# RaulPPelaez/UAMMD

Measured on AMD Instinct MI355X. Metric: particle-steps/s (LJ 1e6, rho*=0.8) + FCM-BDHI steps/s @128^3, 1/2/4/8 GPU, higher is better.
Workload: dtype f32

## Files before the change

### uammd_amd/csrc/fcm.hip

```cpp
#include "ibm.hpp"
#include "celllist.hpp"
#include "rocfft_plans.hpp"
#include "saru.hpp"

#include <cmath>
#include <string>

namespace uammd_hip {

struct PseGreens { float rh, split, eta, shear; bool on; };

struct FcmPrep {
  int4 *origin;
  float *weights;
  float4 *force;
  int *tileOf;
  int *rank;
  int *tileCount;
  int *tileStart;
  int wstride;
  int3 tdim;
  unsigned long long *rec;
  int *ovfTile;
  int cap;
  int *slotCount;
  int *slotCountNext;
  int *slotFlag;
  const float4 *forceById;
};

struct FCM {
  uammd_fcm_parameters par;
  GridT<float> grid;
  IBMKernelDev kern;
  IBMKernelDev kernT{};
  bool haveTorqueKernel = false;
  int nxpad = 0;
  size_t planeReal = 0;
  size_t planeCplx = 0;
  DeviceBuffer gridBuf, gridBufT, interBuf, prepOrigin, prepWeights, prepTileOf, prepRank, prepTileCount, prepTileStart, prepSorted;
  int emVelN = 0;
  DeviceBuffer emVel;
  bool emBin = true;
  bool binnedPending = false;
  const void *binnedPos = nullptr;
  int binnedN = 0;
  bool useTiles = false;
  int3 ntiles{0, 0, 0};
  int3 tdim{8, 8, 8};
  int prepCapN = 0;
  bool tileCountZero = false;
  DeviceBuffer prepRec, prepOvfTile, prepSlotCount;
  bool slotsEnabled = !(getenv("UAMMD_FCM_SLOTS") && atoi(getenv("UAMMD_FCM_SLOTS")) == 0);
  int slotCap = 0;
  int slotParity = 0;
  bool slotPending = false;
  bool slotDirty = true;
  const void *slotPos = nullptr;
  int slotN = 0;
  int slotRefresh = 128;
  bool lastSolveSlots = false;
  int orderN = 0;
  int slotSteps = 0;
  int *slotFlagHost = nullptr, *slotFlagDev = nullptr;
  bool binBySlot = true;
  hipStream_t prepStream = nullptr;
  bool prepStreamSet = false;
  bool forceAtomicSpread = false;
  bool interGather = true;
  int gatherPerWave = 2;
  int spreadWaves = 0;
  bool tileGather = false;
  bool accumulate = false;
  int zTileLog2 = 0;
  bool customFFT = true;
  PseGreens pse{0.f, 0.f, 0.f, 0.f, false};
  RealFFT fft;
  unsigned int seed2 = 0;
  FcmPrep halfPrep{};
  int halfN = 0;
  bool halfPending = false;
  ~FCM() {
    if (slotFlagHost) (void)hipHostFree(slotFlagHost);
  }
};
// ... 176 lines not shown
  const int3 P = compute_support_shift(grid, pi, celli, kern.support);
  const int ox = celli.x - P.x, oy = celli.y - P.y, oz = celli.z - P.z;
  const int slot = pr.tileStart[pr.tileOf[id]] + pr.rank[id];
  float *w = pr.weights + (size_t)pr.wstride * slot;
  const int sx = kern.support.x, sy = kern.support.y, sz = kern.support.z;
  for (int k = sub; k < sx + sy + sz; k += LANES) {
    float v;
    if (k < sx) v = phi_axis(kern, 0, grid.distanceToCellCenter(pi, make_int3(grid.pbc_x(ox + k), celli.y, celli.z)).x);
    else if (k < sx + sy) v = phi_axis(kern, 1, grid.distanceToCellCenter(pi, make_int3(celli.x, grid.pbc_y(oy + k - sx), celli.z)).y);
    else v = phi_axis(kern, 2, grid.distanceToCellCenter(pi, make_int3(celli.x, celli.y, grid.pbc_z(oz + k - sx - sy))).z);
    w[k] = v;
  }
  if (sub) return;
  pr.origin[slot] = make_int4(ox, oy, oz, id);
  float4 fr = force ? force[id] : make_float4(0.f, 0.f, 0.f, 0.f);
  int rel;
  (void)stencil_tile(ox, oy, oz, grid.cellDim, pr.tdim, make_int3(1, 1, 1), &rel);
  fr.w = __int_as_float(rel);
  pr.force[slot] = fr;
}

template <int KIND, int LANES>
__global__ void __launch_bounds__(256) k_fcm_step_prep(float4 *__restrict__ pos, const float *__restrict__ linearV, int N, float dt,
                                                        GridT<float> grid, IBMKernelDev kern, int3 ntiles, FcmPrep pr, int ovfCap) {
  kern.kind = KIND;
  const int gid = blockIdx.x * 256 + threadIdx.x;
  const int s = gid / LANES, sub = gid % LANES;
  const bool live = s < N;
  const bool head = live && sub == 0;
  const int id = live ? pr.origin[s].w : 0;
  float4 p = pos[id];
  if (linearV) {
    p.x = fmaf(linearV[3 * id], dt, p.x);
    p.y = fmaf(linearV[3 * id + 1], dt, p.y);
    p.z = fmaf(linearV[3 * id + 2], dt, p.z);
    if (head) pos[id] = p;
  }
  const real3f pi{p.x, p.y, p.z};
  const int3 celli = grid.getCell(pi);
  const int3 P = compute_support_shift(grid, pi, celli, kern.support);
  const int ox = celli.x - P.x, oy = celli.y - P.y, oz = celli.z - P.z;
  int rel;
  const int t = stencil_tile(ox, oy, oz, grid.cellDim, pr.tdim, ntiles, &rel);
  const int lane = threadIdx.x & 63;
  unsigned long long rem = __ballot(head);
  int cnt = 1, before = 0, lead = lane;
  for (int round = 0; round < 8 && rem; ++round) {
    const int l = __ffsll((unsigned long long)rem) - 1;
    const int t0 = __builtin_amdgcn_readlane(t, l);
    const unsigned long long m = __ballot(head && t == t0) & rem;
    if (head && t == t0 && ((rem >> lane) & 1ull)) {
      cnt = __popcll(m);
      before = __popcll(m & ((1ull << lane) - 1ull));
      lead = l;
    }
    rem &= ~m;
  }
  int got = 0;
  if (head && lane == lead) got = atomicAdd(&pr.slotCount[t], cnt);
  if ((blockIdx.x & 15) == 0 && threadIdx.x < 64) {
// ... 562 lines not shown
        if (wsel[r] >= 0) {
          ax[q] = fmaf(dV, v[q][r].x * wx * wy * wz, ax[q]);
          ay[q] = fmaf(dV, v[q][r].y * wx * wy * wz, ay[q]);
          az[q] = fmaf(dV, v[q][r].z * wx * wy * wz, az[q]);
        }
      }
    }
  }
#pragma unroll
  for (int o2 = 32; o2 > 0; o2 >>= 1) {
#pragma unroll
    for (int q = 0; q < P; ++q) {
      ax[q] += __shfl_xor(ax[q], o2, 64);
      ay[q] += __shfl_xor(ay[q], o2, 64);
      az[q] += __shfl_xor(az[q], o2, 64);
    }
  }
  if (lane == 0) {
#pragma unroll
    for (int q = 0; q < P; ++q) {
      if (slot0 + q >= N) break;
      float *out = vout + 3 * (size_t)o[q].w;
      if (accumulate) { out[0] += ax[q]; out[1] += ay[q]; out[2] += az[q]; } else { out[0] = ax[q]; out[1] = ay[q]; out[2] = az[q]; }
    }
  }
}
template <int P, int SZMAX>
__global__ void __launch_bounds__(64 * kGatherWaves) k_fcm_gather_col(float *__restrict__ vout, const float4 *__restrict__ gi, int N, int3 n,
                                                                      int3 support, float dV, FcmPrep pr, bool accumulate) {
  const int lane = threadIdx.x & 63;
  const int slot0 = ((int)xcd_contiguous_block(blockIdx.x, gridDim.x) * kGatherWaves + (threadIdx.x >> 6)) * P;
  if (slot0 >= N) return;
  const int sx = support.x, sy = support.y, sz = support.z;
  const int ii = lane & 7, jj = lane >> 3;
  const bool col = ii < sx && jj < sy;
  int4 o[P];
  float wl[P];
#pragma unroll
  for (int q = 0; q < P; ++q) {
    const int slot = min(slot0 + q, N - 1);
    o[q] = pr.origin[slot];
    wl[q] = pr.weights[(size_t)pr.wstride * slot + min(lane, sx + sy + sz - 1)];
  }
  float4 g[P][SZMAX];
  float wxy[P];
  const uint planeNodes = (uint)n.x * (uint)n.y;
// ... 24 lines not shown
        const float wz = __builtin_bit_cast(float, __builtin_amdgcn_readlane(__builtin_bit_cast(int, wl[q]), sx + sy + kk));
        const float w = wxy[q] * wz;
        if (col) {
          ax[q] = fmaf(g[q][kk].x, w, ax[q]);
          ay[q] = fmaf(g[q][kk].y, w, ay[q]);
          az[q] = fmaf(g[q][kk].z, w, az[q]);
        }
      }
    }
  }
#pragma unroll
  for (int q = 0; q < P; ++q) {
    ax[q] = wave_total(ax[q]);
    ay[q] = wave_total(ay[q]);
    az[q] = wave_total(az[q]);
  }
  if (lane == 0) {
#pragma unroll
    for (int q = 0; q < P; ++q) {
      if (slot0 + q >= N) break;
      ax[q] *= dV; ay[q] *= dV; az[q] *= dV;
      float *out = vout + 3 * (size_t)o[q].w;
      if (accumulate) { out[0] += ax[q]; out[1] += ay[q]; out[2] += az[q]; } else { out[0] = ax[q]; out[1] = ay[q]; out[2] = az[q]; }
    }
  }
}
template <int S, int SZMAX>
__global__ void __launch_bounds__(64 * kGatherWaves) k_fcm_gather_half(float *__restrict__ vout, const float4 *__restrict__ gi, int N, int3 n,
                                                                       int sz, float dV, FcmPrep pr, bool accumulate) {
  constexpr int R = S * S - 32;
  constexpr int ROUNDS = (R * SZMAX + 31) / 32;
  static_assert(R > 0 && 2 * S + SZMAX <= 32, "supports 6 and 7");
  const int lane = threadIdx.x & 63, h = lane >> 5, l = lane & 31;
  const int slot0 = ((int)xcd_contiguous_block(blockIdx.x, gridDim.x) * kGatherWaves + (threadIdx.x >> 6)) * 2;
  if (slot0 >= N) return;
  const bool valid = slot0 + h < N;
  const int slot = min(slot0 + h, N - 1);
  const int4 o = pr.origin[slot];
  const float wl = pr.weights[(size_t)pr.wstride * slot + min(l, 2 * S + sz - 1)];
  const int jj = l / S, ii = l - S * jj;
  const uint planeNodes = (uint)n.x * (uint)n.y;
  auto wrap = [](int c, int m) { return c < 0 ? c + m : (c >= m ? c - m : c); };
  const uint base = (uint)wrap(o.x + ii, n.x) + (uint)n.x * (uint)wrap(o.y + jj, n.y);
  float4 g[SZMAX];
#pragma unroll
  for (int kk = 0; kk < SZMAX; ++kk)
// ... 33 lines not shown
    const bool rest = kk2[r] >= 0;
    const float w = __shfl(wl, hb + ii2[r], 64) * __shfl(wl, hb + S + jj2[r], 64) * __shfl(wl, hb + 2 * S + (rest ? kk2[r] : 0), 64);
    if (rest) {
      ax = fmaf(g2[r].x, w, ax);
      ay = fmaf(g2[r].y, w, ay);
      az = fmaf(g2[r].z, w, az);
    }
  }
  auto half_sum = [](float x) {
    x += dpp_move<0xB1, 0xf, true>(x);
    x += dpp_move<0x4E, 0xf, true>(x);
    x += dpp_move<0x141, 0xf, true>(x);
    x += dpp_move<0x140, 0xf, true>(x);
    x += dpp_move<0x142, 0xa, false>(x);
    return x;
  };
  ax = half_sum(ax);
  ay = half_sum(ay);
  az = half_sum(az);
  if (l == 31 && valid) {
    ax *= dV; ay *= dV; az *= dV;
    float *out = vout + 3 * (size_t)o.w;
    if (accumulate) { out[0] += ax; out[1] += ay; out[2] += az; } else { out[0] = ax; out[1] = ay; out[2] = az; }
  }
}
static void launch_gather_inter(hipStream_t st, float *vout, const float4 *gi, int N, int3 n, int3 support, float dV, FastDiv dsx,
                                FastDiv dsxy, const FcmPrep &pr, bool accumulate, int perWave = 2, bool packed = false) {
  const size_t nodes = (size_t)n.x * n.y * n.z;
  static const int halfMode = getenv("UAMMD_FCM_GATHER_HALF") ? atoi(getenv("UAMMD_FCM_GATHER_HALF")) : 1;
  if (packed) {
    const int rounds = (support.x * support.y * support.z + 63) / 64;
    const int P = rounds <= 4 ? (perWave >= 4 ? 4 : 2) : 1;
    const dim3 g((N + kGatherWaves * P - 1) / (kGatherWaves * P)), b(64 * kGatherWaves);
#define UH_GIP(RR, PP) hipLaunchKernelGGL((k_fcm_gather_inter<RR, PP, true>), g, b, 0, st, vout, gi, N, n, support, dV, dsx, dsxy, pr, accumulate)
    if (rounds <= 1) UH_GIP(1, 2); else if (rounds <= 2) UH_GIP(2, 2); else if (rounds <= 4) { if (P == 4) UH_GIP(4, 4); else UH_GIP(4, 2); } else UH_GIP(8, 1);
#undef UH_GIP
    return;
  }
  if (halfMode == 2 && perWave >= 0 && support.x == 6 && support.y == 6 && support.z <= 8 && nodes * sizeof(float4) < ((size_t)1 << 32)) {
    const dim3 g((N + kGatherWaves * 2 - 1) / (kGatherWaves * 2)), b(64 * kGatherWaves);
    if (support.z <= 6) hipLaunchKernelGGL((k_fcm_gather_half<6, 6>), g, b, 0, st, vout, gi, N, n, support.z, dV, pr, accumulate);
    else hipLaunchKernelGGL((k_fcm_gather_half<6, 8>), g, b, 0, st, vout, gi, N, n, support.z, dV, pr, accumulate);
    return;
  }
  if (perWave >= 0 && support.x <= 8 && support.y <= 8 && support.z <= 8 && nodes * sizeof(float4) <= ((size_t)128 << 20)) {
    constexpr int P = 2;
// ... 203 lines not shown
  if (t >= total) return;
  const uint tq = lay.divNkx.div((uint)t);
  const uint tz = lay.divNyl.div(tq);
  const int3 cell = make_int3(t - (int)tq * nkx, lay.y0 + (int)(tq - tz * (uint)lay.nyl), (int)tz);
  const int id = cell.x + nkx * (cell.y + nk.y * cell.z);
  const size_t a0 = (size_t)cell.x + (size_t)nkx * (size_t)(cell.y - lay.y0) + lay.zStride * (size_t)cell.z;
  float2 *g1 = g0 + lay.compStride, *g2 = g0 + 2 * lay.compStride;
  C3 in{0.f, 0.f, 0.f, 0.f, 0.f, 0.f};
  if (haveForce && id != 0) {
    const float2 a = g0[a0], b = g1[a0], c = g2[a0];
    in = C3{a.x, a.y, b.x, b.y, c.x, c.y};
  }
  const C3 v = fcm_kspace_node(cell, id, nk, nkx, L, viscosity, haveForce, noisePrefactor, seed1, seed2, pse, in);
  g0[a0] = make_float2(v.xr, v.xi);
  g1[a0] = make_float2(v.yr, v.yi);
  g2[a0] = make_float2(v.zr, v.zi);
}

#include "fcm_fft.hpp"

template <int LOG2TL, int NT, bool P2>
__global__ void __launch_bounds__(NT) k_fft_z_fused(float2 *__restrict__ g, size_t planeC, size_t zStride, int nyl, int y0, int nzArg,
                                                    int3 nk, real3f L, float viscosity, bool haveForce, float noisePrefactor,
                                                    uint seed1, uint seed2, PseGreens pse) {
  extern __shared__ float2 lds[];
  constexpr int TL = 1 << LOG2TL, JG = NT >> LOG2TL, MAXB = 6 * 256 / NT;
  const int nz = fft_len<P2>(nzArg);
  const int LS = nz + 1, nkx = nk.x / 2 + 1;
  float2 *tw = lds, *buf = lds + nz;
  const int tid = threadIdx.x, l = tid & (TL - 1), jg = tid >> LOG2TL;
  const size_t slab = zStride;
  const int q0 = (int)xcd_contiguous_block(blockIdx.x, gridDim.x) * TL, nl = min(TL, nyl * nkx - q0);
  float2 *base = g + q0 + l;
  fft_twiddles<NT>(tw, nz, tid);
  constexpr int NLINES = 3 * TL, QF = 3 * 512 / NT, QL = 2 * 512 / NT;
  const int log2N = 31 - __builtin_clz((unsigned)nz);
  const bool edges = P2 && haveForce && nl == TL && log2N % 3 != 0 && log2N >= 5 && NLINES * (nz >> 2) <= QF * NT &&
                     NLINES * (nz >> 3) <= QL * NT;
  if (edges) {
    const int per = nz >> 2, total = NLINES * per;
    float2 v[QF][4];
#pragma unroll
    for (int q = 0; q < QF; ++q) {
      const int b = tid + q * NT;
      if (b < total) {
        const int j = b / NLINES, line = b - j * NLINES, c = line >> LOG2TL, ll = line & (TL - 1);
        const float2 *src = g + q0 + ll + (size_t)c * planeC + (size_t)j * slab;
#pragma unroll
        for (int r = 0; r < 4; ++r) v[q][r] = src[(size_t)(r * per) * slab];
      }
    }
#pragma unroll
    for (int q = 0; q < QF; ++q) {
      const int b = tid + q * NT;
      if (b < total) {
        const int j = b / NLINES, line = b - j * NLINES;
        fft_butterfly<4, -1>(v[q]);
        float2 *dst = buf + line * LS + 4 * j;
#pragma unroll
        for (int r = 0; r < 4; ++r) dst[r] = v[q][r];
      }
    }
    __syncthreads();
    fft_lds_p2_inner<-1, MAXB, NT>(buf, LS, log2N, NLINES, tw, 1, tid, true, false);
  } else if (haveForce) {
    if (l < nl) {
      const int perC = (nz + JG - 1) / JG;
      staged_copy<12, float2>(0, 3 * perC, 1,
          [&](int e) {
            const int c = e / perC, j = jg + (e - c * perC) * JG;
            return j < nz ? base[(size_t)c * planeC + (size_t)j * slab] : make_float2(0.f, 0.f);
          },
          [&](int e, float2 v) {
            const int c = e / perC, j = jg + (e - c * perC) * JG;
            if (j < nz) buf[(c * nl + l) * LS + j] = v;
          });
    }
    __syncthreads();
    fft_lds<-1, MAXB, NT, P2>(buf, LS, nz, 3 * nl, tw, 1, tid);
  } else
    __syncthreads();
  if (l < nl) {
    const int q = q0 + l, yl = q / nkx, kx = q - yl * nkx, ky = y0 + yl;
    for (int j = jg; j < nz; j += JG) {
      const int3 cell = make_int3(kx, ky, j);
      const int id = kx + nkx * (ky + nk.y * j);
      C3 in{0.f, 0.f, 0.f, 0.f, 0.f, 0.f};
      float2 *px = buf + l * LS + j, *py = buf + (nl + l) * LS + j, *pz = buf + (2 * nl + l) * LS + j;
      if (haveForce) in = C3{px->x, px->y, py->x, py->y, pz->x, pz->y};
      const C3 v = fcm_kspace_node(cell, id, nk, nkx, L, viscosity, haveForce, noisePrefactor, seed1, seed2, pse, in);
      *px = make_float2(v.xr, v.xi);
      *py = make_float2(v.yr, v.yi);
      *pz = make_float2(v.zr, v.zi);
    }
  }
  __syncthreads();
  if (edges) {
    fft_lds_p2_inner<1, MAXB, NT>(buf, LS, log2N, NLINES, tw, 1, tid, false, true);
    const int per = nz >> 3, total = NLINES * per;
#pragma unroll
    for (int q = 0; q < QL; ++q) {
      const int b = tid + q * NT;
      if (b < total) {
        const int j = b / NLINES, line = b - j * NLINES, c = line >> LOG2TL, ll = line & (TL - 1);
        const float2 *p = buf + line * LS + j;
        float2 v[8];
#pragma unroll
        for (int r = 0; r < 8; ++r) v[r] = p[r * per];
#pragma unroll
        for (int r = 1; r < 8; ++r) v[r] = ctw<1>(v[r], tw[j * r]);
        fft_butterfly<8, 1>(v);
        float2 *dst = g + q0 + ll + (size_t)c * planeC + (size_t)j * slab;
#pragma unroll
        for (int r = 0; r < 8; ++r) dst[(size_t)(r * per) * slab] = v[r];
      }
    }
    return;
  }
  fft_lds<1, MAXB, NT, P2>(buf, LS, nz, 3 * nl, tw, 1, tid);
  if (l < nl)
    for (int c = 0; c < 3; ++c)
      for (int j = jg; j < nz; j += JG) base[(size_t)c * planeC + (size_t)j * slab] = buf[(c * nl + l) * LS + j];
}

template <bool ACC>
__global__ void __launch_bounds__(256) k_fcm_half_curl(const float2 *__restrict__ in, float2 *__restrict__ out, size_t planeC,
                                                        int3 nk, real3f L, FastDiv divNkx, FastDiv divNy) {
  const int id = blockIdx.x * 256 + threadIdx.x;
  const int nkx = nk.x / 2 + 1;
  if (id >= nk.z * nk.y * nkx) return;
  const uint tq = divNkx.div((uint)id), tz = divNy.div(tq);
  const int cx = id - (int)tq * nkx, cy = (int)(tq - tz * (uint)nk.y), cz = (int)tz;
  const int3 ik = make_int3(cx - nk.x * (cx >= nkx), cy - nk.y * (cy >= nk.y / 2 + 1), cz - nk.z * (cz >= nk.z / 2 + 1));
  const real3f dk = gradient_fourier(ik, nk, wavevector(ik, L));
  const float2 gx = in[id], gy = in[planeC + id], gz = in[2 * planeC + id];
  const float h = 0.5f;
  float2 cxv = make_float2(h * fmaf(-dk.y, gz.y, dk.z * gy.y), h * fmaf(dk.y, gz.x, -(dk.z * gy.x)));
  float2 cyv = make_float2(h * fmaf(-dk.z, gx.y, dk.x * gz.y), h * fmaf(dk.z, gx.x, -(dk.x * gz.x)));
  float2 czv = make_float2(h * fmaf(-dk.x, gy.y, dk.y * gx.y), h * fmaf(dk.x, gy.x, -(dk.y * gx.x)));
  if (ACC) {
    const float2 ox = out[id], oy = out[planeC + id], oz = out[2 * planeC + id];
    cxv.x += ox.x; cxv.y += ox.y; cyv.x += oy.x; cyv.y += oy.y; czv.x += oz.x; czv.y += oz.y;
  }
  out[id] = cxv;
  out[planeC + id] = cyv;
// ... 67 lines not shown
  else
    hipLaunchKernelGGL((k_fft_x_r2c<false, false>), dim3((nrows + rows - 1) / rows), dim3(kFftThreads), sizeof(float2) * (size_t)(nx + rows * (nh + 1)), st, g,
                       nx, nrows, rows, (const float *)nullptr, (const float *)nullptr, 0);
  const int tiles = (nkx + 15) / 16;
  fft_launch_lines<-1>((float2 *)g, ny, nkx, 3 * nz, st);
  (void)tiles;
  return 0;
}
#ifndef UAMMD_ZG_THREADS
#define UAMMD_ZG_THREADS 256
#endif
static int fcm_fft_z_fused_launch(FCM *f, float2 *g, size_t planeC, size_t zStride, int nyl, int y0, int3 cells, real3f L, bool haveForce,
                                  float noisePrefactor, uint seed2, hipStream_t st) {
  const int nz = cells.z, nkx = cells.x / 2 + 1, lines = nyl * nkx;
  int ltl = nz <= 256 ? 3 : 2;
  if (f->zTileLog2 > 0 && sizeof(float2) * (size_t)(nz + 3 * (1 << f->zTileLog2) * (nz + 1)) <= 64 * 1024) ltl = f->zTileLog2;
  const int tlz = 1 << ltl;
  const size_t ldsz = sizeof(float2) * (size_t)(nz + 3 * tlz * (nz + 1));
  const dim3 gz((lines + tlz - 1) / tlz), bz(512);
#ifndef UAMMD_ZP_THREADS
#define UAMMD_ZP_THREADS 512
#endif
#define UH_ZFUSED(LT, P) hipLaunchKernelGGL((k_fft_z_fused<LT, UAMMD_ZP_THREADS, P>), gz, dim3(UAMMD_ZP_THREADS), ldsz, st, g, planeC, zStride, nyl, y0, nz, cells, L, f->par.viscosity, \
                                         haveForce, noisePrefactor, f->par.seed, seed2, f->pse)
  if (is_pow2(nz)) { if (ltl == 4) UH_ZFUSED(4, true); else if (ltl == 3) UH_ZFUSED(3, true); else UH_ZFUSED(2, true); }
  else {
#define UH_ZFUSED_G(LT) hipLaunchKernelGGL((k_fft_z_fused<LT, UAMMD_ZG_THREADS, false>), gz, dim3(UAMMD_ZG_THREADS), ldsz, st, g, planeC, zStride, nyl, y0, nz, \
                                           cells, L, f->par.viscosity, haveForce, noisePrefactor, f->par.seed, seed2, f->pse)
    if (ltl == 4) UH_ZFUSED_G(4); else if (ltl == 3) UH_ZFUSED_G(3); else UH_ZFUSED_G(2);
#undef UH_ZFUSED_G
  }
#undef UH_ZFUSED
  return 0;
}
static int fcm_fft_z_operator_y(FCM *f, float *g, bool haveForce, float noisePrefactor, hipStream_t st) {
  const int nx = f->grid.cellDim.x, ny = f->grid.cellDim.y, nz = f->grid.cellDim.z, nkx = nx / 2 + 1;
  const real3f L{f->par.boxSize[0], f->par.boxSize[1], f->par.boxSize[2]};
  if (int e = fcm_fft_z_fused_launch(f, (float2 *)g, f->planeCplx, (size_t)ny * nkx, ny, 0, f->grid.cellDim, L, haveForce, noisePrefactor, f->seed2, st)) return e;
  fft_launch_lines<1>((float2 *)g, ny, nkx, 3 * nz, st);
  return 0;
}
static bool fcm_inter_packed(const FCM *f) {
  static const bool on = !(getenv("UAMMD_FCM_PACKED_INTER") && atoi(getenv("UAMMD_FCM_PACKED_INTER")) == 0);
  const size_t nodes = (size_t)f->grid.cellDim.x * f->grid.cellDim.y * f->grid.cellDim.z;
  return on && nodes * sizeof(float4) > ((size_t)128 << 20) && f->gatherPerWave >= 0;
}
static int fcm_fft_inverse_x(FCM *f, float *g, float4 *inter, hipStream_t st, bool packed = false) {
  const int nx = f->grid.cellDim.x, ny = f->grid.cellDim.y, nz = f->grid.cellDim.z, nh = nx / 2;
  const int rows = std::max(1, std::min(8, 2048 / (3 * nh))), nrows = ny * nz;
  if (is_pow2(nx) && is_pow2(ny))
    hipLaunchKernelGGL(k_fft_x_c2r<true>, dim3((nrows + rows - 1) / rows), dim3(kFftThreads), sizeof(float2) * (size_t)(nx + 3 * rows * (nh + 1)), st,
                       g, f->planeReal, (size_t)ny * f->nxpad, ny, nx, nrows, rows, inter, packed ? -1 : 0, (size_t)0);
  else
    hipLaunchKernelGGL(k_fft_x_c2r<false>, dim3((nrows + rows - 1) / rows), dim3(kFftThreads), sizeof(float2) * (size_t)(nx + 3 * rows * (nh + 1)), st,
                       g, f->planeReal, (size_t)ny * f->nxpad, ny, nx, nrows, rows, inter, packed ? -1 : 0, (size_t)0);
  return 0;
}

static int fcm_prepare_tiles(FCM *f, const float *d_pos, const float *d_force, int N, hipStream_t st, FcmPrep *out, bool positionsKept = false) {
  const int nt = f->ntiles.x * f->ntiles.y * f->ntiles.z;
  const int wstride = f->kern.support.x + f->kern.support.y + f->kern.support.z;
  if (f->slotPending) {
    f->slotPending = false;
    f->slotDirty = true;
  }
  f->slotSteps = 0;
  if (f->prepCapN < N) {
    UH_CHECK(hipStreamSynchronize(st));
    f->orderN = 0;
    if (int e = f->prepOrigin.reserve(sizeof(int4) * (size_t)N)) return e;
    if (int e = f->prepWeights.reserve(sizeof(float) * (size_t)wstride * N)) return e;
    if (int e = f->prepSorted.reserve(sizeof(float4) * (size_t)N)) return e;
    if (int e = f->prepTileOf.reserve(sizeof(int) * (size_t)N)) return e;
    if (int e = f->prepRank.reserve(sizeof(int) * (size_t)N)) return e;
    if (int e = f->prepTileCount.reserve(sizeof(int) * (size_t)nt)) return e;
    f->tileCountZero = false;
    if (int e = f->prepTileStart.reserve(sizeof(int) * ((size_t)nt + 1))) return e;
    f->prepCapN = N;
  }
  FcmPrep pr{(int4 *)f->prepOrigin.ptr, (float *)f->prepWeights.ptr, (float4 *)f->prepSorted.ptr,
             (int *)f->prepTileOf.ptr, (int *)f->prepRank.ptr, (int *)f->prepTileCount.ptr,
             (int *)f->prepTileStart.ptr, wstride, f->tdim};
  if (f->prepStreamSet && f->prepStream != st) {
    UH_CHECK(hipStreamSynchronize(f->prepStream));
    f->tileCountZero = false;
  }
  const bool binned = f->binnedPending && positionsKept && f->binnedPos == (const void *)d_pos && f->binnedN == N && f->prepStream == st;
  if (f->binnedPending && !binned) f->tileCountZero = false;
  f->binnedPending = false;
// ... 192 lines not shown
  if (!h) { set_last_error("uammd_fcm_displacements: null argument"); return -1; }
  if (N <= 0) return 0;
  if (!d_pos || (!d_linearVelocity && stage == 0)) { set_last_error("uammd_fcm_displacements: null argument"); return -1; }
  FCM *f = reinterpret_cast<FCM *>(h);
  hipStream_t st = (hipStream_t)stream;
  float *g = (float *)f->gridBuf.ptr;
  const dim3 gp((N + 3) / 4), bp(256);
  const FastDiv dsx = make_fastdiv(f->kern.support.x), dsxy = make_fastdiv(f->kern.support.x * f->kern.support.y);
  if (int e = f->fft.set_stream((void *)st)) return e;
  const size_t zs = (size_t)f->nxpad * f->grid.cellDim.y;
  const bool tiles = f->useTiles && !f->forceAtomicSpread;
  const bool custom = stage == 0 && fcm_custom_fft_usable(f);
  FcmPrep pr{};
  bool slots = false;
  if (half != 2) f->halfPending = false;
  if (half == 2) {
    if (!f->halfPending || f->halfN != N) { set_last_error("uammd_fcm: the second half of a solve without its first"); return -1; }
    pr = f->halfPrep;
    f->halfPending = false;
  } else if (tiles) {
    if (int e = fcm_prepare_best(f, d_pos, d_force, N, st, positionsKept, &pr, &slots)) return e;
  }
  if (half != 2) f->lastSolveSlots = slots;
  if (d_force && half != 2) {
    if (tiles) {
      const int nt = f->ntiles.x * f->ntiles.y * f->ntiles.z;
      const int ww = spread_weight_words(N, f->ntiles, f->kern.support, f->tdim);
      const int sw = spread_waves(N, f->ntiles, f->kern.support, f->tdim, f->spreadWaves);
      const int edge = spread_edge(f->tdim);
      const dim3 sg(nt), sb(64 * sw);
      const size_t lds = spread_lds_bytes(ww, sw, edge);
#define UH_SPREAD(W, S, E) hipLaunchKernelGGL((k_fcm_spread_tile<W, S, E>), sg, sb, lds, st, g, f->grid.cellDim, f->nxpad, f->planeReal, zs, f->kern.support, f->ntiles, pr, ww)
      static const bool specOn = getenv("UAMMD_FCM_NO_SPEC") == nullptr;
      const bool eight = (f->kern.support.x - 2 + f->tdim.x) / f->tdim.x == 1 && (f->kern.support.y - 2 + f->tdim.y) / f->tdim.y == 1 &&
                         (f->kern.support.z - 2 + f->tdim.z) / f->tdim.z == 1;
      static const bool specDense = getenv("UAMMD_FCM_SPEC_DENSE") != nullptr;
      const bool spec = specOn && slots && eight && pr.cap >= 8 * sw && ww / (3 * edge) >= 64 * sw && (sw == 2 || specDense);
#define UH_SPREAD_SPEC(W, E) hipLaunchKernelGGL((k_fcm_spread_tile<W, true, E, true>), sg, sb, lds, st, g, f->grid.cellDim, f->nxpad, f->planeReal, zs, f->kern.support, f->ntiles, pr, ww)
      if (spec) {
        if (sw == 2) { if (edge == kTileMax) UH_SPREAD_SPEC(2, kTileMax); else UH_SPREAD_SPEC(2, kTile); }
        else { if (edge == kTileMax) UH_SPREAD_SPEC(4, kTileMax); else UH_SPREAD_SPEC(4, kTile); }
      }
      else if (edge == kTileMax) {
        if (sw == 2) { if (slots) UH_SPREAD(2, true, kTileMax); else UH_SPREAD(2, false, kTileMax); }
        else { if (slots) UH_SPREAD(4, true, kTileMax); else UH_SPREAD(4, false, kTileMax); }
      } else {
// ... 36 lines not shown
                       f->grid.cellDim, real3f{f->par.boxSize[0], f->par.boxSize[1], f->par.boxSize[2]}, f->par.viscosity,
                       d_force != nullptr, noisePrefactor, f->par.seed, f->seed2, f->pse);
    if (stage == 1) { UH_CHECK(hipGetLastError()); return 0; }
    if (int e = f->fft.inverse(g)) return e;
  }
  const bool interPath = tiles && f->interGather && !(tiles && (f->kern.support.x <= 6 && f->kern.support.y <= 6 && f->kern.support.z <= 6) && f->tileGather);
  if (custom && !interPath) { if (int e = fcm_fft_inverse_x(f, g, nullptr, st)) return e; }
  const bool smallSupport = f->kern.support.x <= 6 && f->kern.support.y <= 6 && f->kern.support.z <= 6;
  if (tiles && smallSupport && f->tileGather)
    hipLaunchKernelGGL(k_fcm_gather_tile, dim3(f->ntiles.x * f->ntiles.y * f->ntiles.z), bp, 0, st, d_linearVelocity,
                       (const float *)g, f->grid.cellDim, f->nxpad, f->planeReal, zs, f->kern.support, f->ntiles,
                       f->grid.cellVolume, dsx, dsxy, pr, f->accumulate);
  else if (tiles && f->interGather) {
    const size_t nodes = (size_t)f->grid.cellDim.x * f->grid.cellDim.y * f->grid.cellDim.z;
    if (int e = f->interBuf.reserve(sizeof(float4) * nodes)) return e;
    const bool packed = custom && fcm_inter_packed(f);
    if (custom) {
      if (int e = fcm_fft_inverse_x(f, g, (float4 *)f->interBuf.ptr, st, packed)) return e;
    } else
      hipLaunchKernelGGL(k_fcm_interleave, dim3((unsigned)((nodes + 255) / 256)), bp, 0, st, (const float *)g, f->grid.cellDim, f->nxpad,
                         f->planeReal, zs, (float4 *)f->interBuf.ptr);
    launch_gather_inter(st, d_linearVelocity, (const float4 *)f->interBuf.ptr, N, f->grid.cellDim, f->kern.support, f->grid.cellVolume,
                        dsx, dsxy, pr, f->accumulate, f->gatherPerWave, packed);
  } else if (tiles)
    hipLaunchKernelGGL(k_fcm_gather_prep, gp, bp, 0, st, d_linearVelocity, (const float *)g, N, f->grid.cellDim, f->nxpad,
                       f->planeReal, zs, f->kern.support, f->grid.cellVolume, dsx, dsxy, pr, f->accumulate);
  else
    hipLaunchKernelGGL((k_fcm_ibm<false>), gp, bp, 0, st, (const float4 *)d_pos, (const float4 *)nullptr,
                       d_linearVelocity, g, N, f->grid, f->nxpad, f->planeReal, zs, f->kern, dsx, dsxy, f->accumulate);
  UH_CHECK(hipGetLastError());
  return 0;
}

int uammd_fcm_displacements_staged(uammd_fcm *h, const float *d_pos, const float *d_force, int N, float temperature,
                                   float prefactor, float *d_linearVelocity, int stage, void *stream) {
  return fcm_displacements_impl(h, d_pos, d_force, N, temperature, prefactor, d_linearVelocity, stage, stream, false);
}

static bool fcm_step_prep_launch(FCM *f, float *d_pos, const float *v, int N, float dt, hipStream_t st, int *rc) {
  *rc = 0;
  if (f->slotFlagHost && f->slotFlagHost[0]) {
    f->slotsEnabled = false;
    return false;
  }
  if (f->slotSteps >= f->slotRefresh) { f->slotSteps = 0; return false; }
  if (v && fcm_entries_scrambled(f, N)) return false;
// ... 14 lines not shown
    if (int e = f->prepRec.reserve(recBytes)) return fail(e);
    if (int e = f->prepOvfTile.reserve(sizeof(int) * (size_t)N)) return fail(e);
    if (int e = f->prepSlotCount.reserve(sizeof(int) * 2 * ((size_t)nt + 2))) return fail(e);
    f->slotCap = cap;
    f->slotDirty = true;
  }
  int *counts = (int *)f->prepSlotCount.ptr;
  int parity;
  if (f->lastSolveSlots && !f->slotDirty) parity = f->slotParity ^ 1;
  else {
    if (hipMemsetAsync(counts, 0, sizeof(int) * 2 * ((size_t)nt + 2), st) != hipSuccess) return fail(-1);
    f->slotDirty = false;
    parity = 0;
  }
  FcmPrep pr{};
  pr.origin = (int4 *)f->prepOrigin.ptr;
  pr.weights = (float *)f->prepWeights.ptr;
  pr.wstride = f->kern.support.x + f->kern.support.y + f->kern.support.z;
  pr.tdim = f->tdim;
  pr.rec = (unsigned long long *)f->prepRec.ptr;
  pr.ovfTile = (int *)f->prepOvfTile.ptr;
  pr.cap = cap;
  pr.slotCount = counts + (size_t)parity * (nt + 2);
#define UH_STEP_PREP(K)                                                                                                                        \
  case K:                                                                                                                                      \
    if (N <= kPrepLanesUpTo)                                                                                                                   \
      hipLaunchKernelGGL((k_fcm_step_prep<K, kPrepLanes>), dim3((unsigned)(((size_t)N * kPrepLanes + 255) / 256)), dim3(256), 0, st, (float4 *)d_pos, v, N, \
                         dt, f->grid, f->kern, f->ntiles, pr, N);                                                                              \
    else                                                                                                                                       \
      hipLaunchKernelGGL((k_fcm_step_prep<K, 1>), dim3((N + 255) / 256), dim3(256), 0, st, (float4 *)d_pos, v, N, dt, f->grid, f->kern,         \
                         f->ntiles, pr, N);                                                                                                    \
    break;
  switch (f->kern.kind) {
    UH_STEP_PREP(kKernelGaussian) UH_STEP_PREP(kKernelPeskin3) UH_STEP_PREP(kKernelPeskin4) UH_STEP_PREP(kKernelConstant)
    UH_STEP_PREP(kKernelBarnettMagland) UH_STEP_PREP(kKernelSixPoint)
    default: return false;
  }
#undef UH_STEP_PREP
  if (hipGetLastError() != hipSuccess) return fail(-1);
  f->slotParity = parity;
  f->slotPending = true;
  f->slotPos = (const void *)d_pos;
  f->slotN = N;
  f->slotSteps++;
  if (f->binnedPending) f->tileCountZero = false;
  f->binnedPending = false;
  return true;
}

int uammd_fcm_step_euler_maruyama(uammd_fcm *h, float *d_pos, const float *d_force, int N, float temperature, float prefactor,
                                  float dt, float *d_linearVelocity, int flags, void *stream) {
  if (!h || (N > 0 && !d_pos)) { set_last_error("uammd_fcm_step_euler_maruyama: null argument"); return -1; }
  if (N <= 0) return 0;
  FCM *f = reinterpret_cast<FCM *>(h);
  hipStream_t st = (hipStream_t)stream;
  float *v = d_linearVelocity;
  if (!v) {
    if (f->emVelN < N) {
      UH_CHECK(hipStreamSynchronize(st));
      if (int e = f->emVel.reserve(sizeof(float) * 3 * (size_t)N)) return e;
      f->emVelN = N;
    }
    v = (float *)f->emVel.ptr;
  }
  if (int e = fcm_displacements_impl(h, d_pos, d_force, N, temperature, prefactor, v, 0, stream, (flags & UAMMD_FCM_STEP_POSITIONS_KEPT) != 0))
    return e;
  const bool tiles = f->useTiles && !f->forceAtomicSpread;
  const bool bin = tiles && f->emBin && f->prepCapN >= N;
  if (bin && f->slotsEnabled) {
    int rc = 0;
    if (fcm_step_prep_launch(f, d_pos, v, N, dt, st, &rc)) return rc;
  }
  FcmPrep pr{};
  if (bin) {
    pr.tileOf = (int *)f->prepTileOf.ptr; pr.rank = (int *)f->prepRank.ptr; pr.tileCount = (int *)f->prepTileCount.ptr;
    pr.origin = (int4 *)f->prepOrigin.ptr;
    pr.tdim = f->tdim;
    if (!f->tileCountZero) {
      UH_CHECK(hipMemsetAsync(pr.tileCount, 0, sizeof(int) * (size_t)(f->ntiles.x * f->ntiles.y * f->ntiles.z), st));
      f->tileCountZero = true;
    }
  }
  hipLaunchKernelGGL(k_fcm_update_bin, dim3((N + 255) / 256), dim3(256), 0, st, (float4 *)d_pos, (const float *)v, N, dt, f->grid, f->ntiles,
                     pr, bin, bin && f->binBySlot, f->kern.support);
  UH_CHECK(hipGetLastError());
  if (bin) { f->binnedPending = true; f->binnedPos = (const void *)d_pos; f->binnedN = N; }
  return 0;
}

int uammd_fcm_set_option(uammd_fcm *h, const char *name, int value) {
  if (!h || !name) { set_last_error("uammd_fcm_set_option: null argument"); return -1; }
  if (std::string(name) == "atomic_spread") { reinterpret_cast<FCM *>(h)->forceAtomicSpread = value != 0; return 0; }
  if (std::string(name) == "bin_ahead") { reinterpret_cast<FCM *>(h)->emBin = value != 0; return 0; }
  if (std::string(name) == "slot_refresh" && value >= 1) { reinterpret_cast<FCM *>(h)->slotRefresh = value; return 0; }
  if (std::string(name) == "slots") { reinterpret_cast<FCM *>(h)->slotsEnabled = value != 0; return 0; }
  if (std::string(name) == "bin_by_slot") { reinterpret_cast<FCM *>(h)->binBySlot = value != 0; return 0; }
  if (std::string(name) == "spread_waves") { reinterpret_cast<FCM *>(h)->spreadWaves = value; return 0; }
  if (std::string(name) == "gather_per_wave") { reinterpret_cast<FCM *>(h)->gatherPerWave = value; return 0; }
  if (std::string(name) == "tile_gather") {
    FCM *f = reinterpret_cast<FCM *>(h);
    const bool fits = f->tdim.x % 2 == 0 && f->tdim.x + f->kern.support.x - 1 <= 16 && f->tdim.y + f->kern.support.y - 1 <= 16 &&
                      f->tdim.z + f->kern.support.z - 1 <= 16;
    f->tileGather = value != 0 && fits;
    return 0;
  }
  if (std::string(name) == "interleaved_gather") { reinterpret_cast<FCM *>(h)->interGather = value != 0; return 0; }
  if (std::string(name) == "z_tile_log2" && (value == 0 || value == 2 || value == 3 || value == 4)) { reinterpret_cast<FCM *>(h)->zTileLog2 = value; return 0; }
  if (std::string(name) == "custom_fft") { reinterpret_cast<FCM *>(h)->customFFT = value != 0; return 0; }
  set_last_error("uammd_fcm_set_option: unknown option %s", name);
  return -1;
}

int uammd_fcm_displacements(uammd_fcm *h, const float *d_pos, const float *d_force, int N, float temperature,
                            float prefactor, float *d_linearVelocity, void *stream) {
  return uammd_fcm_displacements_staged(h, d_pos, d_force, N, temperature, prefactor, d_linearVelocity, 0, stream);
}

// ... 505 lines not shown
```

### uammd_amd/csrc/fcm_fft.hpp

```cpp
#pragma once

constexpr int kFftThreads = 256;
constexpr int kFftMax = 512;

template <bool P2> struct IDivT {
  int d, sh;
  float rcp;
  UH_D explicit IDivT(int dd) : d(dd), sh(31 - __builtin_clz((unsigned)dd)), rcp(1.0f / (float)dd) {}
  UH_D int div(int i) const { return P2 ? (i >> sh) : (int)(((float)i + 0.5f) * rcp); }
  UH_D int mod(int i) const { return P2 ? (i & (d - 1)) : i - __mul24(div(i), d); }
  UH_D int rem(int i, int q) const { return P2 ? (i & (d - 1)) : i - __mul24(q, d); }
};

template <bool P2> UH_D int fft_len(int n) { return P2 ? (1 << (31 - __builtin_clz((unsigned)n))) : n; }

UH_D float2 cadd(float2 a, float2 b) { return make_float2(a.x + b.x, a.y + b.y); }
UH_D float2 csub(float2 a, float2 b) { return make_float2(a.x - b.x, a.y - b.y); }
template <int SIGN> UH_D float2 ctw(float2 a, float2 w) {
  if (SIGN < 0) return make_float2(fmaf(a.x, w.x, -(a.y * w.y)), fmaf(a.x, w.y, a.y * w.x));
  return make_float2(fmaf(a.x, w.x, a.y * w.y), fmaf(a.y, w.x, -(a.x * w.y)));
}

template <int NT = kFftThreads> UH_D void fft_twiddles(float2 *tw, int n, int tid) {
  for (int k = tid; k < n; k += NT) {
// ... 174 lines not shown
    dst[q] = -1;
    if (b < total) {
      const int line = b >> (log2N - LR), j = b & (per - 1), k = j & (Ns - 1);
      const float2 *p = buf + line * LS + j;
      const int t1 = (k << (log2N - log2Ns - LR)) * twStride;
#pragma unroll
      for (int r = 0; r < R; ++r) v[q][r] = p[r * per];
#pragma unroll
      for (int r = 1; r < R; ++r) v[q][r] = ctw<SIGN>(v[q][r], tw[t1 * r]);
      fft_butterfly<R, SIGN>(v[q]);
      dst[q] = line * LS + ((j - k) << LR) + k;
    }
  }
  __syncthreads();
#pragma unroll
  for (int q = 0; q < MAXB; ++q)
    if (dst[q] >= 0) {
#pragma unroll
      for (int r = 0; r < R; ++r) buf[dst[q] + r * Ns] = v[q][r];
    }
  __syncthreads();
}

template <int R, int SIGN, int MAXB, int NT>
UH_D void fft_pass_strided_p2(float2 *buf, int LS, int ES, int log2N, int log2Ns, int nlines, const float2 *tw, int twStride, int tid) {
  constexpr int LR = R == 8 ? 3 : (R == 4 ? 2 : 1);
  const int N = 1 << log2N, per = N >> LR, Ns = 1 << log2Ns, total = nlines << (log2N - LR);
  float2 v[MAXB][R];
  int dst[MAXB];
#pragma unroll
  for (int q = 0; q < MAXB; ++q) {
    const int b = tid + q * NT;
    dst[q] = -1;
    if (b < total) {
      const int line = b % nlines, j = b / nlines, k = j & (Ns - 1);
      const float2 *p = buf + line * LS + j * ES;
      const int t1 = (k << (log2N - log2Ns - LR)) * twStride;
#pragma unroll
      for (int r = 0; r < R; ++r) v[q][r] = p[r * per * ES];
#pragma unroll
      for (int r = 1; r < R; ++r) v[q][r] = ctw<SIGN>(v[q][r], tw[t1 * r]);
      fft_butterfly<R, SIGN>(v[q]);
      dst[q] = line * LS + (((j - k) << LR) + k) * ES;
    }
  }
  __syncthreads();
#pragma unroll
  for (int q = 0; q < MAXB; ++q)
// ... 39 lines not shown
    const int n9 = e3 / 2, r3 = e3 & 1;
    int n12 = 0, n6 = 0, n3 = r3, a2 = e2;
    if (r3) {
      const int plain = passes2(e2) + 1;
      if (e2 >= 2 && passes2(e2 - 2) + 1 < plain) { n12 = 1; n3 = 0; a2 = e2 - 2; }
      else if (e2 >= 1 && passes2(e2 - 1) + 1 < plain) { n6 = 1; n3 = 0; a2 = e2 - 1; }
    }
    n8 = a2 / 3; n4 = 0; n2 = 0;
    if (a2 % 3 == 2) n4 = 1;
    else if (a2 % 3 == 1) { if (n8 > 0) { n8 -= 1; n4 = 2; } else n2 = 1; }
    int Ns = 1;
    for (int a = 0; a < n2; ++a, Ns *= 2) fft_pass<2, SIGN, 2 * MAXB, NT, STRIDED, false>(buf, LS, ES, N, Ns, nlines, tw, twStride, tid);
    for (int a = 0; a < n4; ++a, Ns *= 4) fft_pass<4, SIGN, MAXB, NT, STRIDED, false>(buf, LS, ES, N, Ns, nlines, tw, twStride, tid);
    for (int a = 0; a < n8; ++a, Ns *= 8) fft_pass<8, SIGN, (MAXB + 1) / 2, NT, STRIDED, false>(buf, LS, ES, N, Ns, nlines, tw, twStride, tid);
    for (int a = 0; a < n6; ++a, Ns *= 6) fft_pass<6, SIGN, (4 * MAXB + 5) / 6, NT, STRIDED, false>(buf, LS, ES, N, Ns, nlines, tw, twStride, tid);
    for (int a = 0; a < n12; ++a, Ns *= 12) fft_pass<12, SIGN, (4 * MAXB + 11) / 12, NT, STRIDED, false>(buf, LS, ES, N, Ns, nlines, tw, twStride, tid);
    for (int a = 0; a < n3; ++a, Ns *= 3) fft_pass<3, SIGN, (4 * MAXB + 2) / 3, NT, STRIDED, false>(buf, LS, ES, N, Ns, nlines, tw, twStride, tid);
    for (int a = 0; a < n9; ++a, Ns *= 9) fft_pass<9, SIGN, (4 * MAXB + 8) / 9, NT, STRIDED, false>(buf, LS, ES, N, Ns, nlines, tw, twStride, tid);
    for (int a = 0; a < e5; ++a, Ns *= 5) fft_pass<5, SIGN, (4 * MAXB + 4) / 5, NT, STRIDED, false>(buf, LS, ES, N, Ns, nlines, tw, twStride, tid);
    for (int a = 0; a < e[3]; ++a, Ns *= 7) fft_pass<7, SIGN, (4 * MAXB + 6) / 7, NT, STRIDED, false>(buf, LS, ES, N, Ns, nlines, tw, twStride, tid);
    for (int a = 0; a < e[4]; ++a, Ns *= 11) fft_pass<11, SIGN, (4 * MAXB + 10) / 11, NT, STRIDED, false>(buf, LS, ES, N, Ns, nlines, tw, twStride, tid);
  }
}
template <int SIGN, int MAXB, int NT, bool STRIDED = false>
UH_D void fft_lds_p2_inner(float2 *buf, int LS, int log2N, int nlines, const float2 *tw, int twStride, int tid, bool skipFirst, bool skipLast,
                           int ES = 1) {
  const int m4 = (log2N % 3 == 0) ? 0 : (log2N % 3 == 2 ? 1 : 2);
  int ls = 0;
  bool skip = skipFirst;
  for (int a = 0; a < m4; ++a, ls += 2) {
    if (!skip) {
      if constexpr (STRIDED) fft_pass_strided_p2<4, SIGN, MAXB, NT>(buf, LS, ES, log2N, ls, nlines, tw, twStride, tid);
      else fft_pass_p2<4, SIGN, MAXB, NT>(buf, LS, log2N, ls, nlines, tw, twStride, tid);
    }
    skip = false;
  }
  for (; ls + (skipLast ? 3 : 0) < log2N; ls += 3) {
    if (!skip) {
      if constexpr (STRIDED) fft_pass_strided_p2<8, SIGN, (MAXB + 1) / 2, NT>(buf, LS, ES, log2N, ls, nlines, tw, twStride, tid);
      else fft_pass_p2<8, SIGN, (MAXB + 1) / 2, NT>(buf, LS, log2N, ls, nlines, tw, twStride, tid);
    }
    skip = false;
  }
}
template <int SIGN, int MAXB, int NT, bool P2>
UH_D void fft_lds(float2 *buf, int LS, int N, int nlines, const float2 *tw, int twStride, int tid) {
  fft_lds_any<SIGN, MAXB, NT, false, P2>(buf, LS, 1, N, nlines, tw, twStride, tid);
}
template <int SIGN, int MAXB, int NT, bool P2>
UH_D void fft_lds_strided(float2 *buf, int LS, int ES, int N, int nlines, const float2 *tw, int twStride, int tid) {
  fft_lds_any<SIGN, MAXB, NT, true, P2>(buf, LS, ES, N, nlines, tw, twStride, tid);
}

template <int NT, bool P2> UH_D void fft_untangle_r2c(float2 *buf, int LS, int nh, int nrows, const float2 *tw, int twx, int tid) {
  const int half = (nh + 1) / 2;
  const IDivT<P2> dHalf(half);
  for (int i = tid; i < nrows * half; i += NT) {
    const int r = dHalf.div(i), k = dHalf.rem(i, r);
    float2 *row = buf + r * LS;
    if (k == 0) {
      if ((nh & 1) == 0) {
        const float2 m = row[nh / 2];
// ... 356 lines not shown
```

Baseline: 5.454 billion.

## Cache slot-ordered positions/velocities for step prep and transpose z-FFT LDS layout

```diff
diff --git a/uammd_amd/csrc/fcm.hip b/uammd_amd/csrc/fcm.hip
--- a/uammd_amd/csrc/fcm.hip
+++ b/uammd_amd/csrc/fcm.hip
@@ -27,6 +27,7 @@
   int *slotCountNext;
   int *slotFlag;
   const float4 *forceById;
+  float4 *velEntry;
 };
 
 struct FCM {
@@ -61,6 +62,15 @@
   int slotRefresh = 128;
   bool lastSolveSlots = false;
   int orderN = 0;
+  bool entryCopy = true;
+  DeviceBuffer entryPos, entryVel;
+  int entryCapN = 0;
+  bool entryPosValid = false;
+  const void *entryPosFor = nullptr;
+  int entryPosN = 0;
+  bool wantVelEntry = false;
+  bool velEntryWritten = false;
+  bool zTransposed = true;
   int slotSteps = 0;
   int *slotFlagHost = nullptr, *slotFlagDev = nullptr;
   bool binBySlot = true;
@@ -283,20 +293,26 @@
 
 template <int KIND, int LANES>
 __global__ void __launch_bounds__(256) k_fcm_step_prep(float4 *__restrict__ pos, const float *__restrict__ linearV, int N, float dt,
-                                                        GridT<float> grid, IBMKernelDev kern, int3 ntiles, FcmPrep pr, int ovfCap) {
+                                                        GridT<float> grid, IBMKernelDev kern, int3 ntiles, FcmPrep pr, int ovfCap,
+                                                        float4 *posEntry, const float4 *velEntry, bool posFromEntry) {
   kern.kind = KIND;
   const int gid = blockIdx.x * 256 + threadIdx.x;
   const int s = gid / LANES, sub = gid % LANES;
   const bool live = s < N;
   const bool head = live && sub == 0;
+  const int se = live ? s : 0;
   const int id = live ? pr.origin[s].w : 0;
-  float4 p = pos[id];
+  float4 p = posFromEntry ? posEntry[se] : pos[id];
   if (linearV) {
-    p.x = fmaf(linearV[3 * id], dt, p.x);
-    p.y = fmaf(linearV[3 * id + 1], dt, p.y);
-    p.z = fmaf(linearV[3 * id + 2], dt, p.z);
+    float vx, vy, vz;
+    if (velEntry) { const float4 ve = velEntry[se]; vx = ve.x; vy = ve.y; vz = ve.z; }
+    else { vx = linearV[3 * id]; vy = linearV[3 * id + 1]; vz = linearV[3 * id + 2]; }
+    p.x = fmaf(vx, dt, p.x);
+    p.y = fmaf(vy, dt, p.y);
+    p.z = fmaf(vz, dt, p.z);
     if (head) pos[id] = p;
   }
+  if (head && posEntry) posEntry[s] = p;
   const real3f pi{p.x, p.y, p.z};
   const int3 celli = grid.getCell(pi);
   const int3 P = compute_support_shift(grid, pi, celli, kern.support);
@@ -905,6 +921,7 @@
       if (slot0 + q >= N) break;
       float *out = vout + 3 * (size_t)o[q].w;
       if (accumulate) { out[0] += ax[q]; out[1] += ay[q]; out[2] += az[q]; } else { out[0] = ax[q]; out[1] = ay[q]; out[2] = az[q]; }
+      if (pr.velEntry) pr.velEntry[slot0 + q] = make_float4(ax[q], ay[q], az[q], 0.f);
     }
   }
 }
@@ -975,6 +992,7 @@
       ax[q] *= dV; ay[q] *= dV; az[q] *= dV;
       float *out = vout + 3 * (size_t)o[q].w;
       if (accumulate) { out[0] += ax[q]; out[1] += ay[q]; out[2] += az[q]; } else { out[0] = ax[q]; out[1] = ay[q]; out[2] = az[q]; }
+      if (pr.velEntry) pr.velEntry[slot0 + q] = make_float4(ax[q], ay[q], az[q], 0.f);
     }
   }
 }
@@ -1054,6 +1072,7 @@
     ax *= dV; ay *= dV; az *= dV;
     float *out = vout + 3 * (size_t)o.w;
     if (accumulate) { out[0] += ax; out[1] += ay; out[2] += az; } else { out[0] = ax; out[1] = ay; out[2] = az; }
+    if (pr.velEntry) pr.velEntry[slot] = make_float4(ax, ay, az, 0.f);
   }
 }
 static void launch_gather_inter(hipStream_t st, float *vout, const float4 *gi, int N, int3 n, int3 support, float dV, FastDiv dsx,
@@ -1303,7 +1322,7 @@
 template <int LOG2TL, int NT, bool P2>
 __global__ void __launch_bounds__(NT) k_fft_z_fused(float2 *__restrict__ g, size_t planeC, size_t zStride, int nyl, int y0, int nzArg,
                                                     int3 nk, real3f L, float viscosity, bool haveForce, float noisePrefactor,
-                                                    uint seed1, uint seed2, PseGreens pse) {
+                                                    uint seed1, uint seed2, PseGreens pse, bool transposed) {
   extern __shared__ float2 lds[];
   constexpr int TL = 1 << LOG2TL, JG = NT >> LOG2TL, MAXB = 6 * 256 / NT;
   const int nz = fft_len<P2>(nzArg);
@@ -1313,6 +1332,9 @@
   const size_t slab = zStride;
   const int q0 = (int)xcd_contiguous_block(blockIdx.x, gridDim.x) * TL, nl = min(TL, nyl * nkx - q0);
   float2 *base = g + q0 + l;
+  const bool tr = P2 && transposed;
+  const int zls = tr ? 1 : LS, zes = tr ? 3 * nl : 1;
+  auto zat = [&](int line, int j) { return line * zls + j * zes; };
   fft_twiddles<NT>(tw, nz, tid);
   constexpr int NLINES = 3 * TL, QF = 3 * 512 / NT, QL = 2 * 512 / NT;
   const int log2N = 31 - __builtin_clz((unsigned)nz);
@@ -1337,13 +1359,14 @@
       if (b < total) {
         const int j = b / NLINES, line = b - j * NLINES;
         fft_butterfly<4, -1>(v[q]);
-        float2 *dst = buf + line * LS + 4 * j;
-#pragma unroll
-        for (int r = 0; r < 4; ++r) dst[r] = v[q][r];
+        float2 *dst = buf + zat(line, 4 * j);
+#pragma unroll
+        for (int r = 0; r < 4; ++r) dst[r * zes] = v[q][r];
       }
     }
     __syncthreads();
-    fft_lds_p2_inner<-1, MAXB, NT>(buf, LS, log2N, NLINES, tw, 1, tid, true, false);
+    if (tr) fft_lds_p2_inner<-1, MAXB, NT, true, NLINES>(buf, 1, log2N, NLINES, tw, 1, tid, true, false, NLINES);
+    else fft_lds_p2_inner<-1, MAXB, NT>(buf, LS, log2N, NLINES, tw, 1, tid, true, false);
   } else if (haveForce) {
     if (l < nl) {
       const int perC = (nz + JG - 1) / JG;
@@ -1354,11 +1377,12 @@
           },
           [&](int e, float2 v) {
             const int c = e / perC, j = jg + (e - c * perC) * JG;
-            if (j < nz) buf[(c * nl + l) * LS + j] = v;
+            if (j < nz) buf[zat(c * nl + l, j)] = v;
           });
     }
     __syncthreads();
-    fft_lds<-1, MAXB, NT, P2>(buf, LS, nz, 3 * nl, tw, 1, tid);
+    if (tr) fft_lds_strided<-1, MAXB, NT, P2>(buf, 1, zes, nz, 3 * nl, tw, 1, tid);
+    else fft_lds<-1, MAXB, NT, P2>(buf, LS, nz, 3 * nl, tw, 1, tid);
   } else
     __syncthreads();
   if (l < nl) {
@@ -1367,7 +1391,7 @@
       const int3 cell = make_int3(kx, ky, j);
       const int id = kx + nkx * (ky + nk.y * j);
       C3 in{0.f, 0.f, 0.f, 0.f, 0.f, 0.f};
-      float2 *px = buf + l * LS + j, *py = buf + (nl + l) * LS + j, *pz = buf + (2 * nl + l) * LS + j;
+      float2 *px = buf + zat(l, j), *py = buf + zat(nl + l, j), *pz = buf + zat(2 * nl + l, j);
       if (haveForce) in = C3{px->x, px->y, py->x, py->y, pz->x, pz->y};
       const C3 v = fcm_kspace_node(cell, id, nk, nkx, L, viscosity, haveForce, noisePrefactor, seed1, seed2, pse, in);
       *px = make_float2(v.xr, v.xi);
@@ -1377,17 +1401,18 @@
   }
   __syncthreads();
   if (edges) {
-    fft_lds_p2_inner<1, MAXB, NT>(buf, LS, log2N, NLINES, tw, 1, tid, false, true);
+    if (tr) fft_lds_p2_inner<1, MAXB, NT, true, NLINES>(buf, 1, log2N, NLINES, tw, 1, tid, false, true, NLINES);
+    else fft_lds_p2_inner<1, MAXB, NT>(buf, LS, log2N, NLINES, tw, 1, tid, false, true);
     const int per = nz >> 3, total = NLINES * per;
 #pragma unroll
     for (int q = 0; q < QL; ++q) {
       const int b = tid + q * NT;
       if (b < total) {
         const int j = b / NLINES, line = b - j * NLINES, c = line >> LOG2TL, ll = line & (TL - 1);
-        const float2 *p = buf + line * LS + j;
+        const float2 *p = buf + zat(line, j);
         float2 v[8];
 #pragma unroll
-        for (int r = 0; r < 8; ++r) v[r] = p[r * per];
+        for (int r = 0; r < 8; ++r) v[r] = p[r * per * zes];
 #pragma unroll
         for (int r = 1; r < 8; ++r) v[r] = ctw<1>(v[r], tw[j * r]);
         fft_butterfly<8, 1>(v);
@@ -1398,10 +1423,11 @@
     }
     return;
   }
-  fft_lds<1, MAXB, NT, P2>(buf, LS, nz, 3 * nl, tw, 1, tid);
+  if (tr) fft_lds_strided<1, MAXB, NT, P2>(buf, 1, zes, nz, 3 * nl, tw, 1, tid);
+  else fft_lds<1, MAXB, NT, P2>(buf, LS, nz, 3 * nl, tw, 1, tid);
   if (l < nl)
     for (int c = 0; c < 3; ++c)
-      for (int j = jg; j < nz; j += JG) base[(size_t)c * planeC + (size_t)j * slab] = buf[(c * nl + l) * LS + j];
+      for (int j = jg; j < nz; j += JG) base[(size_t)c * planeC + (size_t)j * slab] = buf[zat(c * nl + l, j)];
 }
 
 template <bool ACC>
@@ -1515,11 +1541,11 @@
 #define UAMMD_ZP_THREADS 512
 #endif
 #define UH_ZFUSED(LT, P) hipLaunchKernelGGL((k_fft_z_fused<LT, UAMMD_ZP_THREADS, P>), gz, dim3(UAMMD_ZP_THREADS), ldsz, st, g, planeC, zStride, nyl, y0, nz, cells, L, f->par.viscosity, \
-                                         haveForce, noisePrefactor, f->par.seed, seed2, f->pse)
+                                         haveForce, noisePrefactor, f->par.seed, seed2, f->pse, f->zTransposed)
   if (is_pow2(nz)) { if (ltl == 4) UH_ZFUSED(4, true); else if (ltl == 3) UH_ZFUSED(3, true); else UH_ZFUSED(2, true); }
   else {
 #define UH_ZFUSED_G(LT) hipLaunchKernelGGL((k_fft_z_fused<LT, UAMMD_ZG_THREADS, false>), gz, dim3(UAMMD_ZG_THREADS), ldsz, st, g, planeC, zStride, nyl, y0, nz, \
-                                           cells, L, f->par.viscosity, haveForce, noisePrefactor, f->par.seed, seed2, f->pse)
+                                           cells, L, f->par.viscosity, haveForce, noisePrefactor, f->par.seed, seed2, f->pse, false)
     if (ltl == 4) UH_ZFUSED_G(4); else if (ltl == 3) UH_ZFUSED_G(3); else UH_ZFUSED_G(2);
 #undef UH_ZFUSED_G
   }
@@ -1558,6 +1584,7 @@
     f->slotDirty = true;
   }
   f->slotSteps = 0;
+  f->entryPosValid = false;
   if (f->prepCapN < N) {
     UH_CHECK(hipStreamSynchronize(st));
     f->orderN = 0;
@@ -1796,6 +1823,8 @@
     if (int e = fcm_prepare_best(f, d_pos, d_force, N, st, positionsKept, &pr, &slots)) return e;
   }
   if (half != 2) f->lastSolveSlots = slots;
+  pr.velEntry = (f->wantVelEntry && tiles && half == 0 && !f->accumulate && f->entryCapN >= N) ? (float4 *)f->entryVel.ptr : nullptr;
+  f->velEntryWritten = false;
   if (d_force && half != 2) {
     if (tiles) {
       const int nt = f->ntiles.x * f->ntiles.y * f->ntiles.z;
@@ -1878,6 +1907,7 @@
                          f->planeReal, zs, (float4 *)f->interBuf.ptr);
     launch_gather_inter(st, d_linearVelocity, (const float4 *)f->interBuf.ptr, N, f->grid.cellDim, f->kern.support, f->grid.cellVolume,
                         dsx, dsxy, pr, f->accumulate, f->gatherPerWave, packed);
+    f->velEntryWritten = pr.velEntry != nullptr;
   } else if (tiles)
     hipLaunchKernelGGL(k_fcm_gather_prep, gp, bp, 0, st, d_linearVelocity, (const float *)g, N, f->grid.cellDim, f->nxpad,
                        f->planeReal, zs, f->kern.support, f->grid.cellVolume, dsx, dsxy, pr, f->accumulate);
@@ -1938,14 +1968,17 @@
   pr.ovfTile = (int *)f->prepOvfTile.ptr;
   pr.cap = cap;
   pr.slotCount = counts + (size_t)parity * (nt + 2);
+  float4 *posEntry = (f->entryCopy && f->entryCapN >= N) ? (float4 *)f->entryPos.ptr : nullptr;
+  const bool posFromEntry = v && posEntry && f->entryPosValid && f->lastSolveSlots && f->entryPosFor == (const void *)d_pos && f->entryPosN == N;
+  const float4 *velEntry = (v && posEntry && f->velEntryWritten) ? (const float4 *)f->entryVel.ptr : nullptr;
 #define UH_STEP_PREP(K)                                                                                                                        \
   case K:                                                                                                                                      \
     if (N <= kPrepLanesUpTo)                                                                                                                   \
       hipLaunchKernelGGL((k_fcm_step_prep<K, kPrepLanes>), dim3((unsigned)(((size_t)N * kPrepLanes + 255) / 256)), dim3(256), 0, st, (float4 *)d_pos, v, N, \
-                         dt, f->grid, f->kern, f->ntiles, pr, N);                                                                              \
+                         dt, f->grid, f->kern, f->ntiles, pr, N, posEntry, velEntry, posFromEntry);                                            \
     else                                                                                                                                       \
       hipLaunchKernelGGL((k_fcm_step_prep<K, 1>), dim3((N + 255) / 256), dim3(256), 0, st, (float4 *)d_pos, v, N, dt, f->grid, f->kern,         \
-                         f->ntiles, pr, N);                                                                                                    \
+                         f->ntiles, pr, N, posEntry, velEntry, posFromEntry);                                                                  \
     break;
   switch (f->kern.kind) {
     UH_STEP_PREP(kKernelGaussian) UH_STEP_PREP(kKernelPeskin3) UH_STEP_PREP(kKernelPeskin4) UH_STEP_PREP(kKernelConstant)
@@ -1958,6 +1991,9 @@
   f->slotPending = true;
   f->slotPos = (const void *)d_pos;
   f->slotN = N;
+  f->entryPosValid = posEntry != nullptr;
+  f->entryPosFor = (const void *)d_pos;
+  f->entryPosN = N;
   f->slotSteps++;
   if (f->binnedPending) f->tileCountZero = false;
   f->binnedPending = false;
@@ -1979,8 +2015,18 @@
     }
     v = (float *)f->emVel.ptr;
   }
-  if (int e = fcm_displacements_impl(h, d_pos, d_force, N, temperature, prefactor, v, 0, stream, (flags & UAMMD_FCM_STEP_POSITIONS_KEPT) != 0))
-    return e;
+  if (f->entryCopy && f->slotsEnabled && f->useTiles && f->entryCapN < N) {
+    UH_CHECK(hipStreamSynchronize(st));
+    f->entryPosValid = false;
+    f->entryCapN = 0;
+    if (int e = f->entryPos.reserve(sizeof(float4) * (size_t)N)) return e;
+    if (int e = f->entryVel.reserve(sizeof(float4) * (size_t)N)) return e;
+    f->entryCapN = N;
+  }
+  f->wantVelEntry = f->entryCopy;
+  const int e = fcm_displacements_impl(h, d_pos, d_force, N, temperature, prefactor, v, 0, stream, (flags & UAMMD_FCM_STEP_POSITIONS_KEPT) != 0);
+  f->wantVelEntry = false;
+  if (e) return e;
   const bool tiles = f->useTiles && !f->forceAtomicSpread;
   const bool bin = tiles && f->emBin && f->prepCapN >= N;
   if (bin && f->slotsEnabled) {
@@ -2009,6 +2055,8 @@
   if (std::string(name) == "atomic_spread") { reinterpret_cast<FCM *>(h)->forceAtomicSpread = value != 0; return 0; }
   if (std::string(name) == "bin_ahead") { reinterpret_cast<FCM *>(h)->emBin = value != 0; return 0; }
   if (std::string(name) == "slot_refresh" && value >= 1) { reinterpret_cast<FCM *>(h)->slotRefresh = value; return 0; }
+  if (std::string(name) == "entry_copy") { FCM *f = reinterpret_cast<FCM *>(h); f->entryCopy = value != 0; f->entryPosValid = false; return 0; }
+  if (std::string(name) == "z_lds_transposed") { reinterpret_cast<FCM *>(h)->zTransposed = value != 0; return 0; }
   if (std::string(name) == "slots") { reinterpret_cast<FCM *>(h)->slotsEnabled = value != 0; return 0; }
   if (std::string(name) == "bin_by_slot") { reinterpret_cast<FCM *>(h)->binBySlot = value != 0; return 0; }
   if (std::string(name) == "spread_waves") { reinterpret_cast<FCM *>(h)->spreadWaves = value; return 0; }
diff --git a/uammd_amd/csrc/fcm_fft.hpp b/uammd_amd/csrc/fcm_fft.hpp
--- a/uammd_amd/csrc/fcm_fft.hpp
+++ b/uammd_amd/csrc/fcm_fft.hpp
@@ -220,8 +220,9 @@
   __syncthreads();
 }
 
-template <int R, int SIGN, int MAXB, int NT>
-UH_D void fft_pass_strided_p2(float2 *buf, int LS, int ES, int log2N, int log2Ns, int nlines, const float2 *tw, int twStride, int tid) {
+template <int R, int SIGN, int MAXB, int NT, int NLC = 0>
+UH_D void fft_pass_strided_p2(float2 *buf, int LS, int ES, int log2N, int log2Ns, int nlinesArg, const float2 *tw, int twStride, int tid) {
+  const int nlines = NLC > 0 ? NLC : nlinesArg;
   constexpr int LR = R == 8 ? 3 : (R == 4 ? 2 : 1);
   const int N = 1 << log2N, per = N >> LR, Ns = 1 << log2Ns, total = nlines << (log2N - LR);
   float2 v[MAXB][R];
@@ -307,7 +308,7 @@
     for (int a = 0; a < e[4]; ++a, Ns *= 11) fft_pass<11, SIGN, (4 * MAXB + 10) / 11, NT, STRIDED, false>(buf, LS, ES, N, Ns, nlines, tw, twStride, tid);
   }
 }
-template <int SIGN, int MAXB, int NT, bool STRIDED = false>
+template <int SIGN, int MAXB, int NT, bool STRIDED = false, int NLC = 0>
 UH_D void fft_lds_p2_inner(float2 *buf, int LS, int log2N, int nlines, const float2 *tw, int twStride, int tid, bool skipFirst, bool skipLast,
                            int ES = 1) {
   const int m4 = (log2N % 3 == 0) ? 0 : (log2N % 3 == 2 ? 1 : 2);
@@ -315,14 +316,14 @@
   bool skip = skipFirst;
   for (int a = 0; a < m4; ++a, ls += 2) {
     if (!skip) {
-      if constexpr (STRIDED) fft_pass_strided_p2<4, SIGN, MAXB, NT>(buf, LS, ES, log2N, ls, nlines, tw, twStride, tid);
+      if constexpr (STRIDED) fft_pass_strided_p2<4, SIGN, MAXB, NT, NLC>(buf, LS, ES, log2N, ls, nlines, tw, twStride, tid);
       else fft_pass_p2<4, SIGN, MAXB, NT>(buf, LS, log2N, ls, nlines, tw, twStride, tid);
     }
     skip = false;
   }
   for (; ls + (skipLast ? 3 : 0) < log2N; ls += 3) {
     if (!skip) {
-      if constexpr (STRIDED) fft_pass_strided_p2<8, SIGN, (MAXB + 1) / 2, NT>(buf, LS, ES, log2N, ls, nlines, tw, twStride, tid);
+      if constexpr (STRIDED) fft_pass_strided_p2<8, SIGN, (MAXB + 1) / 2, NT, NLC>(buf, LS, ES, log2N, ls, nlines, tw, twStride, tid);
       else fft_pass_p2<8, SIGN, (MAXB + 1) / 2, NT>(buf, LS, log2N, ls, nlines, tw, twStride, tid);
     }
     skip = false;
```

New measurement: 5.460 billion (median of 3 runs). About the same (+0.1%).
